# consensus-shipyard/ipc-filecoin-proofs

Hardware: AMD Instinct MI355X
Metric: Merkle proofs verified/sec + HBM GB/s, 1M-receipt synthetic tipset, 1/2/4/8 GPU (higher is better)
Workload: dtype u64; 1 GPU; BASELINE.json configs[2] (the 1M-receipt tipset the metric is quoted on): 1000000 receipts (Amtv0<Receipt> + one Amt<...; receipts_per_gpu=1000000, claims_per_gpu=1000000, witness_blocks_per_gpu=1288038, witness_bytes_per_gpu=439923915, scan_matches=1002, device=AMD Radeon Graphics

## Files before the change

ipc-filecoin-proofs_amd/csrc/kernels/verify_dev.h:

```cpp
#pragma once
#include "claims_dev.h"
#include "event_table.h"
#include "amt_enum.h"
#include "event_table.h"
#include "tipset_ctx.h"
#include "types_dev.h"

namespace ipcfp {


constexpr unsigned long long kEmptySlot64 = ~0ULL;

__device__ __forceinline__ uint32_t exec_find(const unsigned long long* slots, uint32_t mask, const CidKey* keys,
                                              const CidKey& key) {
    const uint64_t h = cid_hash64(key);
    uint32_t s = uint32_t(h >> 32) & mask;
    for (;;) {
        const unsigned long long cur = slots[s];
        if (cur == kEmptySlot64) return kNoBlock;
        if (uint32_t(cur >> 32) == uint32_t(h) && cid_equal(keys[uint32_t(cur)], key)) return uint32_t(cur);
        s = (s + 1) & mask;
    }
}

__device__ __forceinline__ bool ev_trusted(const ipcfp_trust_policy_t& t, long long epoch) {
    if (t.kind == 0) return true;
    if (t.ec_chain_empty) return false;
    return epoch >= t.min_epoch && epoch <= t.max_epoch;
}

__device__ __forceinline__ bool bytes_equal_global(const uint8_t* __restrict__ a, const uint8_t* __restrict__ b, uint32_t n) {
    uint64_t diff = 0;
    uint32_t i = 0;
    typedef unsigned long long u64x2_t __attribute__((ext_vector_type(2)));
    for (; i + 16 <= n; i += 16) {
        u64x2_t x, y;
        __builtin_memcpy(&x, a + i, 16);
        __builtin_memcpy(&y, b + i, 16);
        diff |= (x.x ^ y.x) | (x.y ^ y.y);
    }
    for (; i + 8 <= n; i += 8) {
        uint64_t x, y;
        __builtin_memcpy(&x, a + i, 8);
        __builtin_memcpy(&y, b + i, 8);
        diff |= x ^ y;
    }
    for (; i < n; ++i) diff |= uint64_t(a[i] ^ b[i]);
    return diff == 0;
}

__device__ __forceinline__ uint32_t verify_event_record(const WitnessView& w, const EventClaimPacked& c, const EventRec& e,
                                                        const uint8_t* __restrict__ blob, const ipcfp_event_filter_t& filter,
                                                        bool has_filter) {
    if (e.emitter != c.emitter) return IPCFP_ST_FALSE_EMITTER;
    if (!(e.base_flags & kEvIsLog)) return IPCFP_ST_FALSE_NOT_EVM_LOG;
    const uint32_t nt = uint32_t(e.base_flags >> kEvTopicShift) & 0xffu;
    if (nt != c.n_topics) return IPCFP_ST_FALSE_TOPIC_COUNT;
    const uint8_t* item = w.arena + (e.base_flags & kEvBaseMask);
    const bool case_a = (e.base_flags & kEvCaseA) != 0;
    for (uint32_t i = 0; i < nt; ++i) {
        const uint8_t* claimed = blob + c.topics_off + 33u * i;
        if (!claimed[0]) return IPCFP_ST_FALSE_TOPIC;
        const uint32_t rel = case_a ? uint32_t(e.topic_rel[0]) + 32u * i : uint32_t(e.topic_rel[i & 3u]);
        if (!bytes_equal_global(item + rel, claimed + 1, 32)) return IPCFP_ST_FALSE_TOPIC;
    }
    if (!(c.flags & EC_DATA_MATCHABLE) || c.data_len != e.data_len) return IPCFP_ST_FALSE_DATA;
    if (!bytes_equal_global(item + e.data_rel, blob + c.data_off, c.data_len)) return IPCFP_ST_FALSE_DATA;
    if (has_filter) {
        if (nt < 2) return IPCFP_ST_FALSE_FILTER;
        const uint32_t r1 = case_a ? uint32_t(e.topic_rel[0]) + 32u : uint32_t(e.topic_rel[1]);
        if (!bytes_equal_global(item + e.topic_rel[0], filter.topic0, 32) || !bytes_equal_global(item + r1, filter.topic1, 32))
            return IPCFP_ST_FALSE_FILTER;
    }
    return IPCFP_ST_TRUE;
}

__device__ __forceinline__ uint32_t verify_event_prefix(const EventClaimPacked& c, const TipsetCtxDev& tc,
                                                        const ipcfp_trust_policy_t& trust) {
    if (!(tc.flags & TC_PARENTS_PARSED) || !(tc.flags & TC_CHILD_PARSED)) return IPCFP_ST_ERR_BAD_CLAIM;
    if (!ev_trusted(trust, c.parent_epoch)) return IPCFP_ST_FALSE_UNTRUSTED_PARENT;
    if (!ev_trusted(trust, c.child_epoch)) return IPCFP_ST_FALSE_UNTRUSTED_CHILD;
    if (tc.child_status != IPCFP_ST_TRUE) return tc.child_status;
    if (!tc.parents_match) return IPCFP_ST_FALSE_PARENTS_MISMATCH;
    if (tc.child_height != c.child_epoch) return IPCFP_ST_FALSE_CHILD_EPOCH;
    if (tc.n_parents == 0) return IPCFP_ST_ERR_EMPTY_PARENTS;
    if (tc.parent0_status != IPCFP_ST_TRUE) return tc.parent0_status;
    if (tc.parent0_height != c.parent_epoch) return IPCFP_ST_FALSE_PARENT_EPOCH;
    if (tc.exec_status != IPCFP_ST_TRUE) return tc.exec_status;
    if (!(c.flags & EC_MSG_PARSED)) return IPCFP_ST_ERR_BAD_CLAIM;
    if (tc.exec_inv && c.exec_index < tc.exec_len && cid_equal(tc.exec_keys[tc.exec_inv[c.exec_index]], c.message))
        return IPCFP_ST_TRUE;
    const uint32_t raw = tc.exec_slots ? exec_find(tc.exec_slots, tc.exec_mask, tc.exec_keys, c.message) : kNoBlock;
    if (raw == kNoBlock) return IPCFP_ST_FALSE_MSG_NOT_IN_EXEC;
    if (uint64_t(tc.exec_pos[raw]) != c.exec_index) return IPCFP_ST_FALSE_EXEC_INDEX;
    return IPCFP_ST_TRUE;
}

__device__ __forceinline__ uint32_t verify_event_from_table(const WitnessView& w, const EventClaimPacked& c,
                                                            const TipsetCtxDev& tc, const uint8_t* __restrict__ blob,
                                                            const ipcfp_event_filter_t& filter, bool has_filter,
                                                            ValueLoc* where, bool& settled) {
    settled = false;
    if (!tc.receipt_leaves || !tc.receipt_recs || c.exec_index < tc.receipt_first ||
        c.exec_index - tc.receipt_first >= tc.n_receipt_leaves)
        return kStPending;
    const ReceiptRec rr = tc.receipt_recs[c.exec_index - tc.receipt_first];
    if (rr.kind == RK_WALK) return kStPending;
    settled = true;
    if (rr.kind == RK_NO_EVENTS) return IPCFP_ST_FALSE_NO_EVENTS_ROOT;
    if (rr.kind >= 64) return rr.kind;
    if (c.event_index == ~0ULL) return IPCFP_ST_ERR;
    if (c.event_index >= 64 || !((rr.bitmap >> c.event_index) & 1ull)) return IPCFP_ST_FALSE_NO_EVENT;
    const EventRec e = tc.event_recs[rr.first + __popcll(rr.bitmap & ((1ull << c.event_index) - 1ull))];
    if (where) *where = ValueLoc{rr.block, uint32_t((e.base_flags & kEvBaseMask) - w.off[rr.block]), e.ev_len};
    return verify_event_record(w, c, e, blob, filter, has_filter);
}

__device__ __forceinline__ bool claim_in_bounds(const EventClaimPacked& c, uint32_t n_ctxs, uint64_t blob_len) {
    return c.context < n_ctxs && c.n_topics <= (1u << 20) && uint64_t(c.topics_off) + 33ull * c.n_topics <= blob_len &&
           uint64_t(c.data_off) + c.data_len <= blob_len;
}

}
```

ipc-filecoin-proofs_amd/csrc/kernels/verify_table.hip:

```cpp
#include <hip/hip_runtime.h>

#include "../common.h"
#include "launch.h"
#include "verify_dev.h"

namespace ipcfp {

typedef unsigned long long u64x2_t __attribute__((ext_vector_type(2)));

__device__ __forceinline__ u64x2_t ld16(const uint8_t* __restrict__ p) {
    u64x2_t v;
    __builtin_memcpy(&v, p, 16);
    return v;
}
__device__ __forceinline__ bool differ32(const u64x2_t a[2], const u64x2_t b[2]) {
    return (((a[0].x ^ b[0].x) | (a[0].y ^ b[0].y)) | ((a[1].x ^ b[1].x) | (a[1].y ^ b[1].y))) != 0;
}

struct ClaimedBytes {
    u64x2_t topic[2][2];
    uint32_t flag[2];
    u64x2_t data[2];
};

__device__ __forceinline__ void load_claimed(const EventClaimPacked& c, const uint8_t* __restrict__ blob, ClaimedBytes& p) {
    p = ClaimedBytes{};
    if (c.n_topics >= 1 && c.n_topics <= 2) {
        const uint8_t* q = blob + c.topics_off;
        p.flag[0] = q[0];
        p.topic[0][0] = ld16(q + 1);
        p.topic[0][1] = ld16(q + 17);
        if (c.n_topics == 2) {
            p.flag[1] = q[33];
            p.topic[1][0] = ld16(q + 34);
            p.topic[1][1] = ld16(q + 50);
        }
    }
    if ((c.flags & EC_DATA_MATCHABLE) && c.data_len == 32) {
        p.data[0] = ld16(blob + c.data_off);
        p.data[1] = ld16(blob + c.data_off + 16);
    }
}

__device__ __forceinline__ uint32_t verify_event_record_batched(const WitnessView& w, const EventClaimPacked& c, const EventRec& e,
                                                                const ClaimedBytes& p, const uint8_t* __restrict__ blob,
                                                                const ipcfp_event_filter_t& filter, bool has_filter) {
    if (e.emitter != c.emitter) return IPCFP_ST_FALSE_EMITTER;
    if (!(e.base_flags & kEvIsLog)) return IPCFP_ST_FALSE_NOT_EVM_LOG;
    const uint32_t nt = uint32_t(e.base_flags >> kEvTopicShift) & 0xffu;
    if (nt != c.n_topics) return IPCFP_ST_FALSE_TOPIC_COUNT;
    if (nt > 2) return verify_event_record(w, c, e, blob, filter, has_filter);
    const uint8_t* item = w.arena + (e.base_flags & kEvBaseMask);
    const bool case_a = (e.base_flags & kEvCaseA) != 0;
    const uint32_t rel0 = e.topic_rel[0], rel1 = case_a ? uint32_t(e.topic_rel[0]) + 32u : uint32_t(e.topic_rel[1]);
    const bool data_shape = (c.flags & EC_DATA_MATCHABLE) && c.data_len == e.data_len;
    const bool data_batched = data_shape && c.data_len == 32;
    u64x2_t t0[2] = {}, t1[2] = {}, d[2] = {};
    if (nt >= 1) {
        t0[0] = ld16(item + rel0);
        t0[1] = ld16(item + rel0 + 16);
    }
    if (nt == 2) {
        t1[0] = ld16(item + rel1);
        t1[1] = ld16(item + rel1 + 16);
    }
    if (data_batched) {
        d[0] = ld16(item + e.data_rel);
        d[1] = ld16(item + e.data_rel + 16);
    }
    if (nt >= 1 && (!p.flag[0] || differ32(p.topic[0], t0))) return IPCFP_ST_FALSE_TOPIC;
    if (nt == 2 && (!p.flag[1] || differ32(p.topic[1], t1))) return IPCFP_ST_FALSE_TOPIC;
    if (!data_shape) return IPCFP_ST_FALSE_DATA;
    if (data_batched ? differ32(p.data, d) : !bytes_equal_global(item + e.data_rel, blob + c.data_off, c.data_len))
        return IPCFP_ST_FALSE_DATA;
    if (has_filter) {
        if (nt < 2) return IPCFP_ST_FALSE_FILTER;
        u64x2_t f0[2], f1[2];
        __builtin_memcpy(f0, filter.topic0, 32);
        __builtin_memcpy(f1, filter.topic1, 32);
        if (differ32(t0, f0) || differ32(t1, f1)) return IPCFP_ST_FALSE_FILTER;
    }
    return IPCFP_ST_TRUE;
}

__device__ __forceinline__ uint32_t verify_table_one(const WitnessView& w, const EventClaimPacked& c, const TipsetCtxDev& tc,
                                                     const uint8_t* __restrict__ blob, const ipcfp_trust_policy_t& trust,
                                                     const ipcfp_event_filter_t& filter, bool has_filter, ValueLoc* where) {
    ClaimedBytes p;
    load_claimed(c, blob, p);
    const bool tabulated = tc.receipt_leaves && tc.receipt_recs && c.exec_index >= tc.receipt_first &&
                           c.exec_index - tc.receipt_first < tc.n_receipt_leaves;
    ReceiptRec rr{RK_WALK, 0, 0, kNoBlock, 0};
    if (tabulated) rr = tc.receipt_recs[c.exec_index - tc.receipt_first];
    const uint32_t st = verify_event_prefix(c, tc, trust);
    if (st != IPCFP_ST_TRUE) return st;
    if (!tabulated || rr.kind == RK_WALK) return kStPending;
    if (rr.kind == RK_NO_EVENTS) return IPCFP_ST_FALSE_NO_EVENTS_ROOT;
    if (rr.kind >= 64) return rr.kind;
    if (c.event_index == ~0ULL) return IPCFP_ST_ERR;
    if (c.event_index >= 64 || !((rr.bitmap >> c.event_index) & 1ull)) return IPCFP_ST_FALSE_NO_EVENT;
    const EventRec e = tc.event_recs[rr.first + __popcll(rr.bitmap & ((1ull << c.event_index) - 1ull))];
    if (where) *where = ValueLoc{rr.block, uint32_t((e.base_flags & kEvBaseMask) - w.off[rr.block]), e.ev_len};
    return verify_event_record_batched(w, c, e, p, blob, filter, has_filter);
}

__global__ __launch_bounds__(256) void k_verify_events_table(WitnessView w, const EventClaimPacked* __restrict__ claims, uint32_t n,
                                                             const TipsetCtxDev* __restrict__ ctxs, uint32_t n_ctxs,
                                                             const uint8_t* __restrict__ blob, uint64_t blob_len,
                                                             ipcfp_trust_policy_t trust, ipcfp_event_filter_t filter,
                                                             int has_filter, uint8_t* __restrict__ status,
                                                             ValueLoc* __restrict__ where) {
    const uint32_t t = blockIdx.x * blockDim.x + threadIdx.x;
    const bool live = t < n;
    EventClaimPacked c;
    if (live) c = claims[t];
    else c.context = 0;
    ValueLoc loc{kNoBlock, 0, 0};
    uint32_t st = IPCFP_ST_ERR_BAD_CLAIM;
    const bool inb = live && claim_in_bounds(c, n_ctxs, blob_len);
    const uint32_t ctx0 = __builtin_amdgcn_readfirstlane(inb ? c.context : 0xffffffffu);
    if (__all(!inb || c.context == ctx0)) {
        if (inb) st = verify_table_one(w, c, ctxs[ctx0], blob, trust, filter, has_filter != 0, where ? &loc : nullptr);
    } else if (inb) {
        st = verify_table_one(w, c, ctxs[c.context], blob, trust, filter, has_filter != 0, where ? &loc : nullptr);
    }
    if (!live) return;
    status[t] = uint8_t(st);
    if (where) where[t] = loc;
}

int launch_verify_events_table(ipcfp_ctx* ctx, const WitnessView& w, const EventClaimPacked* claims_d, uint32_t n,
                               const TipsetCtxDev* ctxs_d, uint32_t n_ctxs, const uint8_t* blob_d, uint64_t blob_len,
                               const ipcfp_trust_policy_t& trust, const ipcfp_event_filter_t& filter, int has_filter,
                               uint8_t* status_d, void* where_d) {
    if (n == 0) return IPCFP_OK;
    hipLaunchKernelGGL(k_verify_events_table, dim3(div_up(n, 256)), dim3(256), 0, ctx->stream, w, claims_d, n, ctxs_d, n_ctxs,
                       blob_d, blob_len, trust, filter, has_filter, status_d, static_cast<ValueLoc*>(where_d));
    IPCFP_HIP(ctx, hipGetLastError());
    return IPCFP_OK;
}

}
```

Measured before the change: 1.244 billion proofs/s.

## Add branchless hot path batching guarded loads for table event verification

Adds a branch-free fast path for common claim shapes (up to two topics, 32-byte data). It replaces the early-return check chain with a Verdict ladder and issues all dependent global loads unconditionally through guarded pointers. Loads are grouped into batches so their memory latency overlaps instead of serialising behind control flow. Claims that need the exec-hash fallback or lack a table event are sent to the original cold path, which re-reads the claim. The cost is extra loads from a safe dummy address, higher register pressure, and a second pass when any lane is cold.

```diff
diff --git a/ipc-filecoin-proofs_amd/csrc/kernels/verify_dev.h b/ipc-filecoin-proofs_amd/csrc/kernels/verify_dev.h
--- a/ipc-filecoin-proofs_amd/csrc/kernels/verify_dev.h
+++ b/ipc-filecoin-proofs_amd/csrc/kernels/verify_dev.h
@@ -96,6 +96,49 @@
     return IPCFP_ST_TRUE;
 }
 
+struct EventCtxFacts {
+    uint32_t flags, n_parents, child_status, parents_match, parent0_status, exec_status;
+    long long child_height, parent0_height;
+    const CidKey* exec_keys;
+    const uint32_t* exec_inv;
+    uint64_t exec_len;
+    bool has_receipt_table;
+    uint64_t n_receipt_leaves, receipt_first;
+    const ReceiptRec* receipt_recs;
+    const EventRec* event_recs;
+};
+
+__device__ __forceinline__ EventCtxFacts event_ctx_facts(const TipsetCtxDev& tc) {
+    return EventCtxFacts{tc.flags,        tc.n_parents,      tc.child_status, tc.parents_match,
+                         tc.parent0_status, tc.exec_status,  tc.child_height, tc.parent0_height,
+                         tc.exec_keys,    tc.exec_inv,       tc.exec_len,     tc.receipt_leaves != nullptr && tc.receipt_recs != nullptr,
+                         tc.n_receipt_leaves, tc.receipt_first, tc.receipt_recs, tc.event_recs};
+}
+
+struct Verdict {
+    uint32_t st = IPCFP_ST_TRUE;
+    bool settled = false;
+    __device__ __forceinline__ void rung(bool fails, uint32_t status) {
+        st = (!settled && fails) ? status : st;
+        settled = settled || fails;
+    }
+};
+
+__device__ __forceinline__ void event_prefix_rungs(Verdict& v, const EventClaimPacked& c, const EventCtxFacts& f,
+                                                   const ipcfp_trust_policy_t& trust) {
+    v.rung(!(f.flags & TC_PARENTS_PARSED) || !(f.flags & TC_CHILD_PARSED), IPCFP_ST_ERR_BAD_CLAIM);
+    v.rung(!ev_trusted(trust, c.parent_epoch), IPCFP_ST_FALSE_UNTRUSTED_PARENT);
+    v.rung(!ev_trusted(trust, c.child_epoch), IPCFP_ST_FALSE_UNTRUSTED_CHILD);
+    v.rung(f.child_status != IPCFP_ST_TRUE, f.child_status);
+    v.rung(!f.parents_match, IPCFP_ST_FALSE_PARENTS_MISMATCH);
+    v.rung(f.child_height != c.child_epoch, IPCFP_ST_FALSE_CHILD_EPOCH);
+    v.rung(f.n_parents == 0, IPCFP_ST_ERR_EMPTY_PARENTS);
+    v.rung(f.parent0_status != IPCFP_ST_TRUE, f.parent0_status);
+    v.rung(f.parent0_height != c.parent_epoch, IPCFP_ST_FALSE_PARENT_EPOCH);
+    v.rung(f.exec_status != IPCFP_ST_TRUE, f.exec_status);
+    v.rung(!(c.flags & EC_MSG_PARSED), IPCFP_ST_ERR_BAD_CLAIM);
+}
+
 __device__ __forceinline__ uint32_t verify_event_from_table(const WitnessView& w, const EventClaimPacked& c,
                                                             const TipsetCtxDev& tc, const uint8_t* __restrict__ blob,
                                                             const ipcfp_event_filter_t& filter, bool has_filter,
diff --git a/ipc-filecoin-proofs_amd/csrc/kernels/verify_table.hip b/ipc-filecoin-proofs_amd/csrc/kernels/verify_table.hip
--- a/ipc-filecoin-proofs_amd/csrc/kernels/verify_table.hip
+++ b/ipc-filecoin-proofs_amd/csrc/kernels/verify_table.hip
@@ -1,4 +1,6 @@
 #include <hip/hip_runtime.h>
+
+#include <cstddef>
 
 #include "../common.h"
 #include "launch.h"
@@ -104,6 +106,116 @@
     return verify_event_record_batched(w, c, e, p, blob, filter, has_filter);
 }
 
+typedef const __attribute__((address_space(1))) uint8_t* gbytes_t;
+__device__ __forceinline__ gbytes_t guarded(bool ok, const void* p, const void* safe) {
+    return ok ? (gbytes_t)p : (gbytes_t)safe;
+}
+__device__ __forceinline__ u64x2_t ld16(gbytes_t p) {
+    u64x2_t v;
+    __builtin_memcpy(&v, p, 16);
+    return v;
+}
+__device__ __forceinline__ void batch_end(uint64_t a, uint64_t b = 0, uint64_t c = 0, uint64_t d = 0, uint64_t e = 0) {
+    asm volatile("" ::"v"(a), "v"(b), "v"(c), "v"(d), "v"(e));
+}
+
+static_assert(offsetof(ReceiptRec, first) == 4 && offsetof(ReceiptRec, bitmap) == 8 && offsetof(ReceiptRec, block) == 16,
+              "verify_table_hot reads a ReceiptRec as three words");
+static_assert(offsetof(EventRec, topic_rel) == 16 && offsetof(EventRec, data_rel) == 24 && offsetof(EventRec, ev_len) == 26 &&
+                  offsetof(EventRec, data_len) == 28,
+              "verify_table_hot reads an EventRec as four words");
+
+__device__ __forceinline__ bool hot_shape(const EventClaimPacked& c) {
+    return c.n_topics <= 2 && (!(c.flags & EC_DATA_MATCHABLE) || c.data_len == 32);
+}
+
+__device__ __forceinline__ uint32_t verify_table_hot(const WitnessView& w, const EventClaimPacked& c, const TipsetCtxDev& tc,
+                                                     const uint8_t* __restrict__ blob, const ipcfp_trust_policy_t& trust,
+                                                     const ipcfp_event_filter_t& filter, bool has_filter, bool want_where,
+                                                     const void* safe, ValueLoc& loc, bool& cold) {
+    const EventCtxFacts f = event_ctx_facts(tc);
+    Verdict v;
+    event_prefix_rungs(v, c, f, trust);
+    const bool pre_ok = !v.settled;
+    const bool tabulated = f.has_receipt_table && c.exec_index >= f.receipt_first && c.exec_index - f.receipt_first < f.n_receipt_leaves;
+    uint64_t rw[3];
+    __builtin_memcpy(rw, guarded(tabulated, f.receipt_recs + (c.exec_index - f.receipt_first), safe), 24);
+    const bool inv_ok = pre_ok && f.exec_inv && f.exec_keys && c.exec_index < f.exec_len;
+    uint32_t inv;
+    __builtin_memcpy(&inv, guarded(inv_ok, f.exec_inv + c.exec_index, safe), 4);
+    const bool matchable = (c.flags & EC_DATA_MATCHABLE) != 0;
+    const gbytes_t q0 = guarded(c.n_topics >= 1, blob + c.topics_off, safe);
+    const gbytes_t q1 = guarded(c.n_topics == 2, blob + c.topics_off + 33, safe);
+    const gbytes_t qd = guarded(matchable, blob + c.data_off, safe);
+    ClaimedBytes p;
+    p.flag[0] = q0[0];
+    p.topic[0][0] = ld16(q0 + 1);
+    p.topic[0][1] = ld16(q0 + 17);
+    p.flag[1] = q1[0];
+    p.topic[1][0] = ld16(q1 + 1);
+    p.topic[1][1] = ld16(q1 + 17);
+    p.data[0] = ld16(qd);
+    p.data[1] = ld16(qd + 16);
+    batch_end(rw[0], rw[1], rw[2], inv);
+    const uint32_t rr_kind = uint32_t(rw[0]), rr_first = uint32_t(rw[0] >> 32), rr_block = uint32_t(rw[2]);
+    const uint64_t rr_bitmap = rw[1];
+
+    CidKey key;
+    __builtin_memcpy(&key, guarded(inv_ok, f.exec_keys + inv, safe), 40);
+    const uint32_t bit = uint32_t(c.event_index) & 63u;
+    const bool present = c.event_index < 64 && ((rr_bitmap >> bit) & 1ull);
+    const bool have_event = pre_ok && tabulated && rr_kind == RK_TABLE && f.event_recs && present;
+    const uint32_t slot = rr_first + uint32_t(__popcll(rr_bitmap & ((1ull << bit) - 1ull)));
+    uint64_t ew[4];
+    __builtin_memcpy(ew, guarded(have_event, f.event_recs + slot, safe), 32);
+    uint64_t block_off;
+    __builtin_memcpy(&block_off, guarded(want_where && have_event, w.off + rr_block, safe), 8);
+    batch_end(key.w[0], key.w[1], key.w[2], key.w[3], key.w[4]);
+    batch_end(ew[0], ew[1], ew[2], ew[3], block_off);
+
+    const bool exec_ok = inv_ok && cid_equal(key, c.message);
+    v.rung(!tabulated || rr_kind == RK_WALK, kStPending);
+    v.rung(rr_kind == RK_NO_EVENTS, IPCFP_ST_FALSE_NO_EVENTS_ROOT);
+    v.rung(rr_kind >= 64, rr_kind);
+    v.rung(c.event_index == ~0ULL, IPCFP_ST_ERR);
+    v.rung(!present, IPCFP_ST_FALSE_NO_EVENT);
+    const bool reached = !v.settled;
+    cold = pre_ok && (!exec_ok || (reached && !have_event));
+
+    const uint64_t base_flags = ew[0], e_emitter = ew[1];
+    const uint32_t rel0 = uint32_t(ew[2]) & 0xffffu, rel1_b = uint32_t(ew[2] >> 16) & 0xffffu;
+    const uint32_t data_rel = uint32_t(ew[3]) & 0xffffu, ev_len = uint32_t(ew[3] >> 16) & 0xffffu, e_data_len = uint32_t(ew[3] >> 32);
+    v.rung(e_emitter != c.emitter, IPCFP_ST_FALSE_EMITTER);
+    v.rung(!(base_flags & kEvIsLog), IPCFP_ST_FALSE_NOT_EVM_LOG);
+    const uint32_t nt = uint32_t(base_flags >> kEvTopicShift) & 0xffu;
+    v.rung(nt != c.n_topics, IPCFP_ST_FALSE_TOPIC_COUNT);
+
+    const bool bytes_wanted = have_event && exec_ok && !v.settled;
+    const uint8_t* item = w.arena + (base_flags & kEvBaseMask);
+    const uint32_t rel1 = (base_flags & kEvCaseA) ? rel0 + 32u : rel1_b;
+    const bool data_shape = matchable && c.data_len == e_data_len;
+    const gbytes_t a0 = guarded(bytes_wanted && nt >= 1, item + rel0, safe);
+    const gbytes_t a1 = guarded(bytes_wanted && nt == 2, item + rel1, safe);
+    const gbytes_t ad = guarded(bytes_wanted && data_shape, item + data_rel, safe);
+    const u64x2_t t0[2] = {ld16(a0), ld16(a0 + 16)}, t1[2] = {ld16(a1), ld16(a1 + 16)}, d[2] = {ld16(ad), ld16(ad + 16)};
+
+    v.rung(nt >= 1 && (!p.flag[0] || differ32(p.topic[0], t0)), IPCFP_ST_FALSE_TOPIC);
+    v.rung(nt == 2 && (!p.flag[1] || differ32(p.topic[1], t1)), IPCFP_ST_FALSE_TOPIC);
+    v.rung(!data_shape, IPCFP_ST_FALSE_DATA);
+    v.rung(differ32(p.data, d), IPCFP_ST_FALSE_DATA);
+    u64x2_t f0[2], f1[2];
+    __builtin_memcpy(f0, filter.topic0, 32);
+    __builtin_memcpy(f1, filter.topic1, 32);
+    v.rung(has_filter && nt < 2, IPCFP_ST_FALSE_FILTER);
+    v.rung(has_filter && (differ32(t0, f0) || differ32(t1, f1)), IPCFP_ST_FALSE_FILTER);
+
+    const bool located = reached && have_event;
+    loc.block = located ? rr_block : kNoBlock;
+    loc.off = located ? uint32_t((base_flags & kEvBaseMask) - block_off) : 0u;
+    loc.len = located ? ev_len : 0u;
+    return v.st;
+}
+
 __global__ __launch_bounds__(256) void k_verify_events_table(WitnessView w, const EventClaimPacked* __restrict__ claims, uint32_t n,
                                                              const TipsetCtxDev* __restrict__ ctxs, uint32_t n_ctxs,
                                                              const uint8_t* __restrict__ blob, uint64_t blob_len,
@@ -119,10 +231,29 @@
     uint32_t st = IPCFP_ST_ERR_BAD_CLAIM;
     const bool inb = live && claim_in_bounds(c, n_ctxs, blob_len);
     const uint32_t ctx0 = __builtin_amdgcn_readfirstlane(inb ? c.context : 0xffffffffu);
-    if (__all(!inb || c.context == ctx0)) {
-        if (inb) st = verify_table_one(w, c, ctxs[ctx0], blob, trust, filter, has_filter != 0, where ? &loc : nullptr);
-    } else if (inb) {
-        st = verify_table_one(w, c, ctxs[c.context], blob, trust, filter, has_filter != 0, where ? &loc : nullptr);
+    bool cold = inb;
+    if (ctx0 != 0xffffffffu && __all(!inb || c.context == ctx0)) {
+        if (inb && hot_shape(c)) {
+            ValueLoc hot_loc;
+            bool again;
+            const uint32_t hot_st = verify_table_hot(w, c, ctxs[ctx0], blob, trust, filter, has_filter != 0, where != nullptr,
+                                                     claims + t, hot_loc, again);
+            st = again ? st : hot_st;
+            loc.block = again ? loc.block : hot_loc.block;
+            loc.off = again ? loc.off : hot_loc.off;
+            loc.len = again ? loc.len : hot_loc.len;
+            cold = again;
+        }
+    }
+    if (__any(cold)) {
+        if (cold) {
+            const EventClaimPacked* mine = claims + t;
+            asm volatile("" : "+v"(mine));
+            const EventClaimPacked cc = *mine;
+            ValueLoc cold_loc{kNoBlock, 0, 0};
+            st = verify_table_one(w, cc, ctxs[cc.context], blob, trust, filter, has_filter != 0, &cold_loc);
+            loc = cold_loc;
+        }
     }
     if (!live) return;
     status[t] = uint8_t(st);
```

After: 1.289 billion proofs/s (median of 6 runs). 1.04x the previous value.
